# CederGroupHub/chgnet

Measured on AMD Instinct MI355X. Metric: structures/s (energy+force+stress) on batched ~50-atom crystals, higher is better.
Workload: dtype f32; 1 GPU; 1024 x LiMnO2 5x1x1 (40 atoms, sigma=0.01 frac perturbation) per GPU, task efs; structures_per_gpu=1024, atoms=40960, directed_bonds=3535504, angles=4125764, bond_graph_nodes=213755, weights=random-init 0.3.0 architecture (tests/golden/weights_seed0.npz), parallelism=structures sharded over 1 GPU(s), RCCL all-gather of energies only, process_group_ranks=1, energies_in_all_gather=1024, comm=none (single rank)

## Files before the change

### chgnet_amd/_lib.py

```python

from __future__ import annotations

import ctypes
import os

c_int_p = ctypes.POINTER(ctypes.c_int32)
c_float_p = ctypes.POINTER(ctypes.c_float)

TASK_BITS = {"e": 1, "f": 2, "s": 4, "m": 8}

EXPORTED_SYMBOLS = (
    "chg_abi_version", "chg_device_count", "chg_weights_required", "chg_engine_create", "chg_engine_destroy", "chg_last_error",
    "chg_batch_upload", "chg_batch_build", "chg_batch_build_predict", "chg_debug_fetch_i32", "chg_batch_update_geometry", "chg_batch_free", "chg_batch_device_bytes",
    "chg_predict", "chg_synchronize", "chg_batch_download", "chg_timer_start", "chg_timer_stop_ms",
    "chg_profile_enable", "chg_profile_reset", "chg_profile_count", "chg_profile_read",
    "chg_debug_fetch", "chg_test_rows_gemm", "chg_test_split_gemm",
    "chg_engine_set_memory_limit", "chg_engine_memory_info", "chg_batch_bytes_required",
    "chg_stream_copy", "chg_backward", "chg_engine_build_stats", "chg_engine_update_weights",
    "chg_engine_set_graph_search", "chg_engine_cell_stats",
    "chg_comm_unique_id", "chg_comm_create", "chg_comm_all_gather_f32", "chg_comm_all_reduce_sum_f32", "chg_comm_barrier",
    "chg_comm_destroy", "chg_comm_last_error",
    "chg_comm_all_gather_f32_device", "chg_comm_all_reduce_sum_f32_device", "chg_comm_reserve", "chg_comm_info",
    "chg_backward_allreduce", "chg_batch_all_gather_energy", "chg_engine_stream", "chg_engine_device",
    "chg_host_alloc", "chg_host_free",
    "chg_relax_create", "chg_relax_run", "chg_relax_download", "chg_relax_free", "chg_test_relax_step",
    "chg_relax_create_lbfgs", "chg_test_lbfgs_step",
    "chg_md_create", "chg_md_run", "chg_md_download", "chg_md_free", "chg_test_md_step",
    "chg_md_create_langevin", "chg_test_md_step_langevin",
    "chg_md_create_nhc", "chg_md_download_nhc", "chg_test_md_step_nhc",
    "chg_md_create_nhc_flex", "chg_md_download_vg", "chg_test_md_step_nhc_flex",
    "chg_hessian_vector", "chg_hessian_vector_strain",
# ... 173 lines not shown
    lib.chg_batch_all_gather_energy.argtypes = [vp, vp, vp, ctypes.c_int64, c_float_p]
    lib.chg_engine_stream.argtypes = [vp]
    lib.chg_engine_stream.restype = ctypes.c_void_p
    lib.chg_engine_device.argtypes = [vp]
    lib.chg_engine_update_weights.argtypes = [vp, c_float_p]
    lib.chg_batch_download.argtypes = [vp, vp, ctypes.POINTER(OutHost)]
    lib.chg_timer_start.argtypes = [vp]
    lib.chg_timer_stop_ms.argtypes = [vp, c_float_p]
    lib.chg_stream_copy.argtypes = [vp, ctypes.c_int64, ctypes.c_int, c_float_p]
    lib.chg_profile_enable.argtypes = [vp, ctypes.c_int]
    lib.chg_profile_reset.argtypes = [vp]
    lib.chg_profile_count.argtypes = [vp]
    lib.chg_profile_read.argtypes = [vp, ctypes.c_int, ctypes.c_char_p, ctypes.c_int, ctypes.POINTER(ctypes.c_int64), ctypes.POINTER(ctypes.c_double)]
    lib.chg_debug_fetch.argtypes = [vp, vp, ctypes.c_char_p, c_float_p, ctypes.c_int64, ctypes.POINTER(ctypes.c_int64)]
    lib.chg_test_rows_gemm.argtypes = [vp, c_float_p, c_float_p, c_float_p, c_float_p, ctypes.c_int, ctypes.c_int, ctypes.c_int]
    lib.chg_test_split_gemm.argtypes = [vp, c_float_p, c_float_p, c_float_p, ctypes.c_int, ctypes.c_int, ctypes.c_int]
    dp = ctypes.POINTER(ctypes.c_double)
    lib.chg_relax_create.argtypes = [vp, ctypes.POINTER(StructsHost), ctypes.POINTER(RelaxParams), ctypes.POINTER(vp)]
    lib.chg_relax_run.argtypes = [vp, vp, ctypes.c_int32, c_int_p]
    lib.chg_relax_download.argtypes = [vp, vp, ctypes.POINTER(RelaxOutHost)]
    lib.chg_relax_free.argtypes = [vp, vp]
    lib.chg_test_relax_step.argtypes = [vp, ctypes.POINTER(RelaxParams), ctypes.c_int32, c_int_p, dp, dp, dp, c_int_p, c_float_p, c_float_p,
                                        c_float_p, c_float_p, dp, dp]
    lib.chg_relax_create_lbfgs.argtypes = [vp, ctypes.POINTER(StructsHost), ctypes.POINTER(RelaxParams), ctypes.POINTER(LbfgsParams),
                                           ctypes.POINTER(vp)]
    lib.chg_test_lbfgs_step.argtypes = [vp, ctypes.POINTER(RelaxParams), ctypes.POINTER(LbfgsParams), ctypes.c_int32, c_int_p, dp, dp, dp, dp, dp,
                                        dp, dp, c_int_p, c_float_p, c_float_p, c_float_p, c_float_p, ctypes.c_int32, dp, dp, c_int_p]
    lib.chg_md_create.argtypes = [vp, ctypes.POINTER(StructsHost), dp, dp, ctypes.POINTER(MdParams), ctypes.POINTER(vp)]
    lib.chg_md_run.argtypes = [vp, vp, ctypes.c_int32]
    lib.chg_md_download.argtypes = [vp, vp, ctypes.POINTER(MdOutHost)]
    lib.chg_md_free.argtypes = [vp, vp]
# ... 34 lines not shown
```

### chgnet_amd/csrc/engine.hip

```cpp

#include "engine_internal.h"
#include <cstring>

namespace chgh {

template <int UNROLL>
__global__ __launch_bounds__(256) void k_stream_copy(const f32x4* __restrict__ src, f32x4* __restrict__ dst, size_t n) {
  const size_t stride = (size_t)gridDim.x * blockDim.x;
  size_t i = (size_t)blockIdx.x * blockDim.x + threadIdx.x;
  for (; i + (UNROLL - 1) * stride < n; i += UNROLL * stride) {
    f32x4 v[UNROLL];
#pragma unroll
    for (int u = 0; u < UNROLL; ++u) v[u] = __builtin_nontemporal_load(src + i + u * stride);
#pragma unroll
    for (int u = 0; u < UNROLL; ++u) __builtin_nontemporal_store(v[u], dst + i + u * stride);
  }
  for (; i < n; i += stride) dst[i] = src[i];
}

template <bool NT>
__global__ __launch_bounds__(256) void k_stream_copy_seg(const f32x4* __restrict__ src, f32x4* __restrict__ dst, size_t n) {
  constexpr size_t SEG = 1024;
  const size_t nseg = n / SEG;
  for (size_t sgm = blockIdx.x; sgm < nseg; sgm += gridDim.x) {
// ... 542 lines not shown
  float *dx = nullptr, *dw = nullptr, *db = nullptr, *dy = nullptr;
  HIP_TRY(eng, hipMalloc(&dx, sizeof(float) * (size_t)rows * k));
  HIP_TRY(eng, hipMalloc(&dw, sizeof(float) * (size_t)nout * k));
  HIP_TRY(eng, hipMalloc(&db, sizeof(float) * (size_t)nout));
  HIP_TRY(eng, hipMalloc(&dy, sizeof(float) * (size_t)rows * nout));
  HIP_TRY(eng, hipMemcpy(dx, x, sizeof(float) * (size_t)rows * k, hipMemcpyHostToDevice));
  HIP_TRY(eng, hipMemcpy(dw, wt, sizeof(float) * (size_t)nout * k, hipMemcpyHostToDevice));
  if (bias) HIP_TRY(eng, hipMemcpy(db, bias, sizeof(float) * (size_t)nout, hipMemcpyHostToDevice));
  int s = rows_gemm(eng, "test_gemm", k, nout, dx, k, nullptr, dw, bias ? db : nullptr, nullptr, 0, dy, nout, nullptr, rows, 0);
  if (s == CHG_OK && hipStreamSynchronize(eng->stream) != hipSuccess) { eng->err = "test gemm failed"; s = CHG_EHIP; }
  if (s == CHG_OK) hipMemcpy(y, dy, sizeof(float) * (size_t)rows * nout, hipMemcpyDeviceToHost);
  hipFree(dx); hipFree(dw); hipFree(db); hipFree(dy);
  return s;
}

int chg_test_split_gemm(chg_engine* eng, const float* x, const float* w, float* y, int rows, int f, int mode) {
  if (!eng || !x || !w || !y || rows <= 0 || (f != D && f != 2 * D) || mode < 0 || mode > 3) return CHG_EINVAL;
  HIP_TRY(eng, hipSetDevice(eng->device));
  const int kin = (mode & 1) ? f : D, nout = (mode & 1) ? D : f;
  float *dx = nullptr, *dw = nullptr, *dy = nullptr;
  HIP_TRY(eng, hipMalloc(&dx, sizeof(float) * (size_t)rows * kin));
  HIP_TRY(eng, hipMalloc(&dw, sizeof(float) * (size_t)f * D));
  HIP_TRY(eng, hipMalloc(&dy, sizeof(float) * (size_t)rows * nout));
  HIP_TRY(eng, hipMemcpy(dx, x, sizeof(float) * (size_t)rows * kin, hipMemcpyHostToDevice));
  HIP_TRY(eng, hipMemcpy(dw, w, sizeof(float) * (size_t)f * D, hipMemcpyHostToDevice));
  hipStream_t st = eng->stream;
  switch (mode * 2 + (f == D ? 0 : 1)) {
    case 0: launch_test_split<0, D>(st, dx, dw, dy, rows); break;
    case 1: launch_test_split<0, 2 * D>(st, dx, dw, dy, rows); break;
    case 2: launch_test_split<1, D>(st, dx, dw, dy, rows); break;
// ... 15 lines not shown
```

### chgnet_amd/csrc/engine_internal.h

```cpp
#pragma once

#include "chgnet_hip.h"

#include <hip/hip_runtime.h>

#include <algorithm>
#include <cmath>
#include <cstdint>
#include <cstdio>
#include <cstdlib>
#include <cstring>
#include <functional>
#include <map>
#include <mutex>
#include <string>
#include <unordered_map>
#include <vector>

#include "mfma_tile.h"
#include "mfma_split.h"
#include "kernels_conv.h"
#include "kernels_angle_w.h"
#include "kernels_angle_blk.h"
#include "kernels_embed.h"
// ... 24 lines not shown
  }
  std::string& slot() const { return texts()[this]; }
  ErrText& operator=(const std::string& v) { slot() = v; return *this; }
  ErrText& operator=(const char* v) { slot() = v; return *this; }
  operator std::string() const { return slot(); }
  const char* c_str() const { return slot().c_str(); }
  ~ErrText() { texts().erase(this); }
};
inline std::string operator+(const char* a, const ErrText& b) { return std::string(a) + std::string(b); }
inline std::string operator+(const std::string& a, const ErrText& b) { return a + std::string(b); }
inline std::string operator+(const ErrText& a, const char* b) { return std::string(a) + b; }
inline std::string operator+(const ErrText& a, const std::string& b) { return std::string(a) + b; }

struct ProfEntry { std::string label; int64_t launches = 0; double ms = 0.0; };
struct PendingEvent { int entry; hipEvent_t start, stop; };

struct chg_engine {
  int device = 0;
  hipStream_t stream = nullptr;
  chg_model_desc desc{};
  float* d_weights = nullptr;
  Weights w{};
  float* d_images = nullptr;
  const float* p_elem = nullptr;
  const float* img_ac_fwd[2][MAX_CONV] = {};
  const float* img_ac_bwd_rm[MAX_CONV] = {};
  const float* img_angle[2][2 * MAX_CONV] = {};
  ErrText err;
  hipEvent_t t0 = nullptr, t1 = nullptr;
  bool profiling = false;
// ... 10 lines not shown
  bool force_wide = false;
  char* scratch = nullptr;
  size_t scratch_bytes = 0, scratch_wanted = 0;
  char* h_stage = nullptr;
  size_t h_stage_bytes = 0;
  char* h_out = nullptr;
  size_t h_out_bytes = 0;
  int num_cus = 256;
  bool spec_builds = true;
  int last_N = 0, last_Ed = 0, last_A = 0, last_Eb = 0;
  double last_r_atom = 0.0, last_r_bond = 0.0;
  long n_spec_builds = 0, n_spec_overflows = 0, n_cell_builds = 0, n_cell_fallbacks = 0;
  int graph_search = 0;
  int cell_min_atoms = 2048;
  size_t memory_limit = 0;
};

struct Train2;

struct chg_batch {
  int B = 0, N = 0, Ed = 0, Eu = 0, A = 0, Eb = 0, L = 0;
  char* arena = nullptr;
  size_t arena_bytes = 0;
  int *z, *atom_owner, *atom_off, *e_center, *e_nbr, *e_d2u, *e_owner, *e_rev, *p_center, *p_nbr, *u_u2d, *u_bnode, *bn_und, *a_ctr, *a_b1c, *a_b2c, *a_d1, *a_d2;
  float *frac, *lattice, *e_image;
  float* cart;
  f32x4 *ev, *eu;
  float *hb0, *wag, *wbgc;
  float* atom[MAX_CONV + 1];
  float* hbc[MAX_CONV + 1];
// ... 194 lines not shown
```

### chgnet_amd/csrc/engine_predict.hip

```cpp
#include "engine_internal.h"

#include "kernels_geom.h"
#include "kernels_angle_fa.h"
#include "kernels_chain.h"

namespace chgh {


struct Cursor {
  const float* base;
  size_t pos = 0;
  const float* take(size_t n) {
    pos += (4 - pos % 4) % 4;
    const float* p = base + pos;
    pos += n;
    return p;
  }
};

void take_gated_tail(Cursor& c, GatedW& g, const float*& w2c_t, const float*& w2g_t) {
  g.w2c = c.take(D * D); g.b2c = c.take(D); g.w2g = c.take(D * D); g.b2g = c.take(D);
  w2c_t = c.take(D * D); w2g_t = c.take(D * D);
}
void take_ln(Cursor& c, GatedW& g) {
// ... 73 lines not shown
constexpr int EMBED_GRID_MULT = 2;

int grid_for(int rows, int max_blocks, int block_rows) {
  int ntiles = (rows + block_rows - 1) / block_rows;
  int g = std::min(ntiles, max_blocks);
  if (g >= 8) g &= ~7;
  return std::max(g, 1);
}

int tile_grid(chg_engine* eng, int rows, int block_rows) {
  const int ntiles = (rows + block_rows - 1) / block_rows;
  const int mult = ntiles <= 4 * eng->num_cus ? 1 : TILE_GRID_MULT;
  return std::max(1, std::min((ntiles + 7) & ~7, mult * eng->num_cus));
}

template <int K, int NOUT, int PARTS = 1>
int launch_rows_gemm(chg_engine* eng, const char* label, const RowsGemm& p) {
  if (p.rows <= 0) return CHG_OK;
  LaunchScope ls(eng, label);
  const size_t lds = rows_gemm_lds<K, NOUT, PARTS>();
  hipLaunchKernelGGL((k_rows_gemm<K, NOUT, PARTS>), dim3(grid_for(p.rows, 4 * eng->num_cus)), dim3(BLOCK), lds, eng->stream, p);
  HIP_TRY(eng, hipGetLastError());
  return CHG_OK;
}

constexpr int SMALL_GEMM_ROWS = 32768;
constexpr int SMALL_GEMM_COLS = 16;
template <int K, int PARTS>
int launch_rows_gemm_cols(chg_engine* eng, const char* label, RowsGemm p, int n_out, int n_out_first) {
  if (p.rows <= 0) return CHG_OK;
  p.col_blocks = n_out / SMALL_GEMM_COLS; p.blocks1 = n_out_first / SMALL_GEMM_COLS;
  LaunchScope ls(eng, label);
  hipLaunchKernelGGL((k_rows_gemm<K, SMALL_GEMM_COLS, PARTS>), dim3(grid_for(p.rows, 4 * eng->num_cus), p.col_blocks), dim3(BLOCK),
                     (rows_gemm_lds<K, SMALL_GEMM_COLS, PARTS>()), eng->stream, p);
  HIP_TRY(eng, hipGetLastError());
  return CHG_OK;
}

int rows_gemm(chg_engine* eng, const char* label, int K, int NOUT, const float* X, int ldx, const int* in_idx, const float* Wt,
              const float* bias, const float* resid, int ldr, float* Y, int ldy, const int* out_idx, int rows, int accumulate) {
  RowsGemm p{X, ldx, in_idx, Wt, bias, resid, ldr, Y, ldy, out_idx, rows, accumulate, nullptr, 0, 0, 0, 0};
  if (rows <= SMALL_GEMM_ROWS && K == 64 && (NOUT == 64 || NOUT == 128)) return launch_rows_gemm_cols<64, 1>(eng, label, p, NOUT, NOUT);
  if (rows <= SMALL_GEMM_ROWS && K == 128 && NOUT == 64) return launch_rows_gemm_cols<128, 1>(eng, label, p, NOUT, NOUT);
  if (K == 64 && NOUT == 64) return launch_rows_gemm<64, 64>(eng, label, p);
  if (K == 64 && NOUT == 128) return launch_rows_gemm<64, 128>(eng, label, p);
  if (K == 128 && NOUT == 64) return launch_rows_gemm<128, 64>(eng, label, p);
  eng->err = "rows_gemm: unsupported shape";
  return CHG_EINVAL;
}

int rows_gemm_out2(chg_engine* eng, const char* label, const float* X, const int* in_idx, const float* Wt, const float* Wt2,
                   const float* bias, float* Y, int ldy, int rows) {
  RowsGemm p{X, D, in_idx, Wt, bias, nullptr, 0, Y, ldy, nullptr, rows, 0, Wt2, 0, 2 * D, 0, 0};
  if (rows <= SMALL_GEMM_ROWS) return launch_rows_gemm_cols<64, 1>(eng, label, p, 4 * D, 2 * D);
  return launch_rows_gemm<64, 128, 2>(eng, label, p);
}
int rows_gemm_in2(chg_engine* eng, const char* label, const float* X, int ldx, const float* Wt, const float* Wt2, float* Y,
                  const int* out_idx, int rows, int accumulate) {
  RowsGemm p{X, ldx, nullptr, Wt, nullptr, nullptr, 0, Y, D, out_idx, rows, accumulate, Wt2, 2 * D, 0, 0, 0};
  if (rows <= SMALL_GEMM_ROWS) return launch_rows_gemm_cols<128, 2>(eng, label, p, D, D);
  return launch_rows_gemm<128, 64, 2>(eng, label, p);
}

struct MultiGemm {
  RowsGemmN g{};
  int max_rows = 0;
  void add(RowsGemm p, int n_out, int n_out_first) {
    p.col_blocks = n_out / SMALL_GEMM_COLS; p.blocks1 = n_out_first / SMALL_GEMM_COLS;
    g.p[g.n++] = p;
    max_rows = std::max(max_rows, p.rows);
  }
};
template <int K>
int launch_rows_gemm_multi(chg_engine* eng, const char* label, const MultiGemm& m) {
  int blocks = 0;
  for (int i = 0; i < m.g.n; ++i) blocks += m.g.p[i].col_blocks;
  LaunchScope ls(eng, label);
  hipLaunchKernelGGL((k_rows_gemm_multi<K, SMALL_GEMM_COLS>), dim3(grid_for(m.max_rows, 4 * eng->num_cus), blocks), dim3(BLOCK),
                     (rows_gemm_lds<K, SMALL_GEMM_COLS, (K == 128 ? 2 : 1)>()), eng->stream, m.g);
  HIP_TRY(eng, hipGetLastError());
  return CHG_OK;
}
static bool small_rows(int rows) { return rows > 0 && rows <= SMALL_GEMM_ROWS; }

int zero(chg_engine* eng, void* p, size_t bytes) {
  if (bytes == 0) return CHG_OK;
  LaunchScope ls(eng, "memset");
  HIP_TRY(eng, hipMemsetAsync(p, 0, bytes, eng->stream));
  return CHG_OK;
}





static bool addr32_mode(const chg_batch* b) {
  constexpr size_t HARD = (size_t)1 << 32;
  static const int forced = [] { const char* e = std::getenv("CHGNET_ADDR_MODE"); return e ? std::atoi(e) : 0; }();
// ... 136 lines not shown
  return CHG_OK;
}

int atomconv_bwd(chg_engine* eng, chg_batch* b, int l) {
  const ACW& w = eng->w.ac[l];
  if (b->Ed == 0) return CHG_OK;
  TRY(rows_gemm(eng, "gemm_Gagg", 64, 64, b->Ga, D, nullptr, w.w_out_t, nullptr, nullptr, 0, b->GA, D, nullptr, b->N, 0));
  TRY(atomconv_bwd_kernel(eng, b, l));
  if (l > 0) TRY(rows_gemm_in2(eng, "gemm_GP", b->GP_l[l], 4 * D, w.w_cn_t, w.w_cn_t + 2 * D * D, b->Ga, nullptr, b->N, 1));
  return CHG_OK;
}

int angle_tables(chg_engine* eng, chg_batch* b, int slot, const float* atom, const float* hbc, const float* w_bij, const float* w_ctr, const float* b1,
                 int p_layer = -1) {
  float *S = b->Sl[slot], *R = b->Rl[slot];
  if (small_rows(b->N) && small_rows(b->Eb)) {
    MultiGemm m;
    m.add(RowsGemm{atom, D, nullptr, w_ctr, b1, nullptr, 0, S, 2 * D, nullptr, b->N, 0, nullptr, 0, 0, 0, 0}, 2 * D, 2 * D);
    m.add(RowsGemm{hbc, D, nullptr, w_bij, nullptr, nullptr, 0, R, 4 * D, nullptr, b->Eb, 0, w_bij + 2 * D * D, 0, 2 * D, 0, 0}, 4 * D, 2 * D);
    if (p_layer >= 0 && b->Ed > 0) {
      m.add(atomconv_p_problem(eng, b, p_layer), 4 * D, 2 * D);
      b->p_table_done = p_layer;
    }
    return launch_rows_gemm_multi<64>(eng, m.g.n == 3 ? "gemm_SRP" : "gemm_SR", m);
  }
  TRY(rows_gemm(eng, "gemm_S", 64, 128, atom, D, nullptr, w_ctr, b1, nullptr, 0, S, 2 * D, nullptr, b->N, 0));
  return rows_gemm_out2(eng, "gemm_R", hbc, nullptr, w_bij, w_bij + 2 * D * D, nullptr, R, 4 * D, b->Eb);
}

AngleArgs angle_args(chg_batch* b, int slot, const float* ang, const float* w_ang, const GatedW& g, float* out) {
  AngleArgs a{};
// ... 68 lines not shown

int bondconv_fwd(chg_engine* eng, chg_batch* b, int l) {
  const BCW& w = eng->w.bc[l];
  TRY(angle_tables(eng, b, l, b->atom[l + 1], b->hbc[l], w.w_bij, w.w_ctr, w.b1, l + 1));
  TRY((launch_angle<true, false>(eng, "bondconv_fwd", b, angle_args(b, l, b->ang[l], w.w_ang, w.g, b->aggB_l[l]))));
  return rows_gemm(eng, "gemm_out", 64, 64, b->aggB_l[l], D, nullptr, w.w_out, w.b_out, b->hbc[l], D, b->hbc[l + 1], D, nullptr, b->Eb, 0);
}

int angleupd_fwd(chg_engine* eng, chg_batch* b, int l) {
  const AUW& w = eng->w.au[l];
  TRY(angle_tables(eng, b, b->L + l, b->atom[l + 1], b->hbc[l + 1], w.w_bij, w.w_ctr, w.b1));
  return launch_angle<false, false, FWD_WAVES>(eng, "angleupd_fwd", b, angle_args(b, b->L + l, b->ang[l], w.w_ang, w.g, b->ang[l + 1]));
}

int angle_table_grads(chg_engine* eng, chg_batch* b, int slot, const float* w_bij_t, const float* w_ctr_t) {
  if (small_rows(b->N) && small_rows(b->Eb)) {
    MultiGemm m;
    m.add(RowsGemm{b->GR_l[slot], 4 * D, nullptr, w_bij_t, nullptr, nullptr, 0, b->Gb, D, b->bn_und, b->Eb, 1, w_bij_t + 2 * D * D, 2 * D, 0, 0, 0}, D, D);
    m.add(RowsGemm{b->GS_l[slot], 2 * D, nullptr, w_ctr_t, nullptr, nullptr, 0, b->Ga, D, nullptr, b->N, 1, nullptr, 0, 0, 0, 0}, D, D);
    return launch_rows_gemm_multi<128>(eng, "gemm_GRS", m);
  }
  TRY(rows_gemm_in2(eng, "gemm_GR", b->GR_l[slot], 4 * D, w_bij_t, w_bij_t + 2 * D * D, b->Gb, b->bn_und, b->Eb, 1));
  return rows_gemm(eng, "gemm_GS", 128, 64, b->GS_l[slot], 2 * D, nullptr, w_ctr_t, nullptr, nullptr, 0, b->Ga, D, nullptr, b->N, 1);
}

int bondconv_bwd(chg_engine* eng, chg_batch* b, int l) {
  const BCW& w = eng->w.bc[l];
  TRY(rows_gemm(eng, "gemm_Gagg", 64, 64, b->Gb, D, b->bn_und, w.w_out_t, nullptr, nullptr, 0, b->Gagg, D, nullptr, b->Eb, 0));
  TRY((launch_angle<true, true>(eng, "bondconv_bwd", b, angle_args(b, l, b->ang[l], w.w_ang, w.g, nullptr))));
  return angle_table_grads(eng, b, l, w.w_bij_t, w.w_ctr_t);
}
// ... 451 lines not shown
  return CHG_OK;
}

void register_names(chg_batch* b) {
  auto& m = b->named;
  m.clear();
  const size_t N = b->N, Ed = b->Ed, Eu = b->Eu, A = b->A, Eb = b->Eb, B = b->B;
  m["cart"] = {b->cart, 3 * N};
  m["ev"] = {reinterpret_cast<const float*>(b->ev), 4 * Ed};
  m["eu"] = {reinterpret_cast<const float*>(b->eu), 4 * Ed};
  m["hb0"] = {b->hb0, Eu * D}; m["wag"] = {b->wag, Eu * D}; m["wbgc"] = {b->wbgc, Eb * D};
  for (int l = 0; l <= b->L; ++l) m["atom" + std::to_string(l)] = {b->atom[l], N * D};
  for (int l = 0; l < b->L; ++l) m["hbc" + std::to_string(l)] = {b->hbc[l], Eb * D};
  for (int l = 0; l < b->L - 1; ++l) m["ang" + std::to_string(l)] = {b->ang[l], A * D};
  for (int l = 0; l < b->L; ++l) { m["P" + std::to_string(l)] = {b->Pl[l], N * 4 * D}; m["Q" + std::to_string(l)] = {b->Ql[l], Eu * 2 * D}; }
  m["agg"] = {b->agg_l[b->L - 1], N * D}; m["aggB"] = {b->aggB_l[0], Eb * D};
  m["Ga"] = {b->Ga, N * D}; m["GA"] = {b->GA, N * D}; m["Gb"] = {b->Gb, Eu * D}; m["Gwag"] = {b->Gwag, Eu * D};
  m["Gwbgc"] = {b->Gwbgc, Eb * D}; m["Gang"] = {b->Gang, A * D}; m["GP"] = {b->GP_l[0], N * 4 * D}; m["GQ"] = {b->GQ, Eu * 2 * D};
  m["GR"] = {b->GR_l[0], Eb * 4 * D}; m["GS"] = {b->GS_l[0], N * 2 * D}; m["Grk"] = {b->Grk, Eu}; m["Gu"] = {b->Gu, 4 * Ed};
  m["virial"] = {b->virial, 9 * B}; m["volume"] = {b->volume, B};
  m["frac"] = {b->frac, 3 * N}; m["lattice"] = {b->lattice, 9 * B}; m["e_image"] = {b->e_image, 3 * Ed};
  auto& mi = b->named_i32;
  mi.clear();
  mi["z"] = {b->z, N}; mi["atom_owner"] = {b->atom_owner, N}; mi["atom_off"] = {b->atom_off, B + 1};
  mi["e_center"] = {b->e_center, Ed}; mi["e_nbr"] = {b->e_nbr, Ed}; mi["e_d2u"] = {b->e_d2u, Ed}; mi["e_owner"] = {b->e_owner, Ed};
  mi["e_rev"] = {b->e_rev, Ed}; mi["p_center"] = {b->p_center, Ed}; mi["p_nbr"] = {b->p_nbr, Ed};
  mi["u_u2d"] = {b->u_u2d, Eu}; mi["u_bnode"] = {b->u_bnode, Eu}; mi["bn_und"] = {b->bn_und, Eb};
  mi["a_ctr"] = {b->a_ctr, A}; mi["a_b1c"] = {b->a_b1c, A}; mi["a_b2c"] = {b->a_b2c, A}; mi["a_d1"] = {b->a_d1, A}; mi["a_d2"] = {b->a_d2, A};
  mi["win_flag"] = {b->win.flag, 4}; mi["win_q_a"] = {b->win.q_a, A}; mi["win_q_ctr"] = {b->win.q_ctr, A}; mi["win_na"] = {b->win.na, N + 1};
  mi["win_aoff"] = {b->win.aoff, N + 1}; mi["win_q_ab1"] = {b->win.q_ab1, A}; mi["win_q_ab2"] = {b->win.q_ab2, A};
  mi["win_next_atom"] = {b->win.next_atom, A ? N : 0};
  mi["blk_tiles"] = {b->blk_tiles, b->blk_cap ? (size_t)1 : 0}; mi["blk_a"] = {b->blk_a, (size_t)b->blk_cap * TILE_ROWS};
  mi["blk_b1c"] = {b->blk_b1c, (size_t)b->blk_cap * TILE_ROWS}; mi["blk_b2c"] = {b->blk_b2c, (size_t)b->blk_cap * TILE_ROWS};
  mi["blk_ctr"] = {b->blk_ctr, (size_t)b->blk_cap * TILE_ROWS}; mi["blk_desc"] = {b->blk_desc, (size_t)b->blk_cap};
  mi["win_wave_head"] = {b->win.wave_head, A ? (size_t)WIN_MAX_GRID * WAVES : 0}; mi["win_xatom"] = {b->win.xatom, (size_t)WIN_MAX_GRID / 8 + 1};
}


int predict_set_lds(chg_engine* eng) {
  int s;
  if ((s = set_lds(eng, k_rows_gemm<64, 64>, rows_gemm_lds<64, 64>()))) return s;
  if ((s = set_lds(eng, k_rows_gemm<64, 128>, rows_gemm_lds<64, 128>()))) return s;
  if ((s = set_lds(eng, k_rows_gemm<128, 64>, rows_gemm_lds<128, 64>()))) return s;
  if ((s = set_lds(eng, k_rows_gemm<64, SMALL_GEMM_COLS, 1>, (rows_gemm_lds<64, SMALL_GEMM_COLS, 1>())))) return s;
  if ((s = set_lds(eng, k_rows_gemm_multi<64, SMALL_GEMM_COLS>, (rows_gemm_lds<64, SMALL_GEMM_COLS, 1>())))) return s;
  if ((s = set_lds(eng, k_rows_gemm_multi<128, SMALL_GEMM_COLS>, (rows_gemm_lds<128, SMALL_GEMM_COLS, 2>())))) return s;
  if ((s = set_lds(eng, k_rows_gemm<128, SMALL_GEMM_COLS, 1>, (rows_gemm_lds<128, SMALL_GEMM_COLS, 1>())))) return s;
  if ((s = set_lds(eng, k_rows_gemm<128, SMALL_GEMM_COLS, 2>, (rows_gemm_lds<128, SMALL_GEMM_COLS, 2>())))) return s;
  if ((s = set_lds(eng, (k_rows_gemm<64, 128, 2>), (rows_gemm_lds<64, 128, 2>())))) return s;
  if ((s = set_lds(eng, (k_rows_gemm<128, 64, 2>), (rows_gemm_lds<128, 64, 2>())))) return s;
  if ((s = set_lds(eng, k_atomconv_fwd<FWD_WAVES>, (atomconv_lds<FWD_WAVES, false, true>())))) return s;
  if ((s = set_lds(eng, k_atomconv_bwd<false>, acb_fused_lds()))) return s;
  if ((s = set_lds(eng, k_angleupd_fwd_a<>, angle_fa_lds()))) return s;
  if ((s = set_lds(eng, (k_atomconv_fwd<FWD_WAVES, true>), (atomconv_lds<FWD_WAVES, false, true>())))) return s;
  if ((s = set_lds(eng, (k_atomconv_bwd<false, true>), acb_fused_lds()))) return s;
  if ((s = set_lds(eng, k_angleupd_fwd_a<true>, angle_fa_lds()))) return s;
  if ((s = set_lds(eng, (k_angle_bwd_w<true, false, false, true>), angle_w_lds<true>()))) return s;
  if ((s = set_lds(eng, (k_angle_bwd_w<true, false, true, true>), angle_w_lds<true>()))) return s;
  if ((s = set_lds(eng, (k_angle_bwd_w<false, false, false, true>), angle_w_lds<false>()))) return s;
  if ((s = set_lds(eng, (k_angle<true, false, WAVES, false, true>), angle_lds<true>()))) return s;
  if ((s = set_lds(eng, k_angle_bwd_blk<true>, angle_blk_lds<true>()))) return s;
  if ((s = set_lds(eng, k_angle_bwd_blk<false>, angle_blk_lds<false>()))) return s;
  if ((s = set_lds(eng, k_angle_bwd_w<true>, angle_w_lds<true>()))) return s;
  if ((s = set_lds(eng, k_angle_bwd_w<false>, angle_w_lds<false>()))) return s;
  if ((s = set_lds(eng, (k_angle_bwd_w<true, true>), angle_w_lds<true>()))) return s;
// ... 23 lines not shown
```

### chgnet_amd/csrc/kernels_conv.h

```cpp
#pragma once

#include "mfma_tile.h"
#include "mfma_split.h"

namespace chg {

constexpr int TS = 2 * D + PAD;
constexpr int WS = D + PAD;
constexpr int TILE_FLOATS = TILE_ROWS * TS;
constexpr int VEC_SLOTS = 6;
constexpr int IMG64 = 1024, IMG128 = 2048;
constexpr int angle_split(bool hidden, bool bwd) { return (hidden && bwd) ? 2 : 1; }

struct GatedW {
  const float *w2c, *b2c, *w2g, *b2g, *ln1_g, *ln1_b, *ln2_g, *ln2_b;
};

__device__ __forceinline__ void stage_gated_vecs(float* vecs, const GatedW& gw, bool hidden, int tid) {
  if (hidden) {
    stage_vector(vecs + 0 * D, gw.b2c, D, tid);
    stage_vector(vecs + 1 * D, gw.b2g, D, tid);
  }
  stage_vector(vecs + 2 * D, gw.ln1_g, D, tid);
  stage_vector(vecs + 3 * D, gw.ln1_b, D, tid);
// ... 352 lines not shown
#pragma unroll
  for (int i = 0; i < 3; ++i) {
    if (i >= g.n) return;
    if (y < g.p[i].col_blocks) {
      if (K == 128 && g.p[i].x2_off > 0) rows_gemm_body<K, NOUT, (K == 128 ? 2 : 1)>(g.p[i], y);
      else rows_gemm_body<K, NOUT, 1>(g.p[i], y);
      return;
    }
    y -= g.p[i].col_blocks;
  }
}

template <int K, int NOUT, int PARTS = 1>
constexpr size_t rows_gemm_lds() {
  return sizeof(float) * (PARTS * NOUT * (K + PAD) + NOUT + WAVES * TILE_ROWS * ((K > NOUT ? K : NOUT) + PAD));
}

struct AtomConvArgs {
  const float* P;
  const float* Q;
  const float* wag;
  const int *e_center, *e_nbr, *e_d2u;
  int n_edges;
  GatedW gw;
  const float *hb0, *hbc;
  const int* u_bnode;
  const float *w_bond, *q_bias;
  float* Qout;
  const float* image;
  float* agg;
// ... 707 lines not shown
```

### chgnet_amd/engine.py

```python

from __future__ import annotations

import ctypes
import weakref

import numpy as np

from chgnet_amd import _lib
from chgnet_amd.graph.structure import atomic_numbers_of
from chgnet_amd.pack import D, PackedBatch, PackedWeights, _check_z, pack_batch


def _fp(a: np.ndarray):
    return a.ctypes.data_as(_lib.c_float_p)


def _ip(a: np.ndarray):
    return a.ctypes.data_as(_lib.c_int_p)


class PreparedStructures:

    __slots__ = ("n_struct", "z", "atom_off", "frac", "lattice")

# ... 325 lines not shown
        got = ctypes.c_int64()
        self._check(self.lib.chg_debug_fetch(self.handle, batch.handle, name.encode(), _fp(dst), n, ctypes.byref(got)))
        if got.value != n:
            raise RuntimeError(f"debug_fetch({name}): expected {n} floats, device buffer has {got.value}")
        return dst[:n].reshape(shape)

    def test_split_gemm(self, x: np.ndarray, w: np.ndarray, mode: int) -> np.ndarray:
        x = np.ascontiguousarray(x, np.float32)
        w = np.ascontiguousarray(w, np.float32)
        f = w.shape[0]
        assert w.shape[1] == 64 and x.shape[1] == (f if mode & 1 else 64)
        y = np.empty((x.shape[0], 64 if mode & 1 else f), np.float32)
        self._check(self.lib.chg_test_split_gemm(self.handle, _fp(x), _fp(w), _fp(y), x.shape[0], f, int(mode)))
        return y

    def test_rows_gemm(self, x: np.ndarray, wt: np.ndarray, bias: np.ndarray | None) -> np.ndarray:
        x = np.ascontiguousarray(x, np.float32)
        wt = np.ascontiguousarray(wt, np.float32)
        rows, k = x.shape
        nout = wt.shape[0]
        y = np.empty((rows, nout), np.float32)
        b = np.ascontiguousarray(bias, np.float32) if bias is not None else None
        self._check(self.lib.chg_test_rows_gemm(self.handle, _fp(x), _fp(wt), _fp(b) if b is not None else None, _fp(y), rows, k, nout))
        return y
```

### include/chgnet_hip.h

```cpp
#ifndef CHGNET_HIP_H
#define CHGNET_HIP_H

#include <stdint.h>

#ifdef __cplusplus
extern "C" {
#endif

typedef enum {
  CHG_OK = 0,
  CHG_EINVAL = -1,
  CHG_EHIP = -2,
  CHG_ENOMEM = -3,
  CHG_ENODEV = -4,
  CHG_EUNSUPPORTED = -5,
  CHG_ERANGE = -6
} chg_status;

enum {
  CHG_TASK_E = 1u,
  CHG_TASK_F = 2u,
  CHG_TASK_S = 4u,
  CHG_TASK_M = 8u
};
// ... 101 lines not shown
int chg_batch_download(chg_engine* eng, chg_batch* batch, const chg_out_host* out);

int chg_timer_start(chg_engine* eng);
int chg_timer_stop_ms(chg_engine* eng, float* elapsed_ms);

int chg_stream_copy(chg_engine* eng, int64_t bytes, int iters, float* ms_per_iter);

int chg_profile_enable(chg_engine* eng, int on);
int chg_profile_reset(chg_engine* eng);
int chg_profile_count(chg_engine* eng);
int chg_profile_read(chg_engine* eng, int i, char* label, int label_cap, int64_t* launches, double* total_ms);

int chg_debug_fetch(chg_engine* eng, chg_batch* batch, const char* name, float* dst, int64_t capacity, int64_t* n_written);

int chg_test_rows_gemm(chg_engine* eng, const float* x, const float* wt, const float* bias, float* y, int rows, int k, int nout);
int chg_test_split_gemm(chg_engine* eng, const float* x, const float* w, float* y, int rows, int f, int mode);

enum { CHG_RELAX_RUNNING = 0, CHG_RELAX_CONVERGED = 1, CHG_RELAX_MAX_STEPS = 2, CHG_RELAX_NONFINITE = 3 };
typedef struct chg_relax_params {
  double fmax;
  int32_t max_steps, relax_cell;
  double dt, maxstep, dtmax, finc, fdec, astart, fa;
  int32_t nmin;
  double exp_cell_factor;
  double r_atom, r_bond, numerical_tol;
  double stress_weight;
} chg_relax_params;
typedef struct chg_relax chg_relax;
typedef struct chg_relax_out_host {
  double* frac;
// ... 153 lines not shown
```

Before: 41040 structures/s.

## Add software-pipelined persistent rows GEMM kernel for large row counts

```diff
diff --git a/chgnet_amd/_lib.py b/chgnet_amd/_lib.py
--- a/chgnet_amd/_lib.py
+++ b/chgnet_amd/_lib.py
@@ -14,7 +14,7 @@
     "chg_batch_upload", "chg_batch_build", "chg_batch_build_predict", "chg_debug_fetch_i32", "chg_batch_update_geometry", "chg_batch_free", "chg_batch_device_bytes",
     "chg_predict", "chg_synchronize", "chg_batch_download", "chg_timer_start", "chg_timer_stop_ms",
     "chg_profile_enable", "chg_profile_reset", "chg_profile_count", "chg_profile_read",
-    "chg_debug_fetch", "chg_test_rows_gemm", "chg_test_split_gemm",
+    "chg_debug_fetch", "chg_test_rows_gemm", "chg_test_split_gemm", "chg_test_set_gemm_stream_rows",
     "chg_engine_set_memory_limit", "chg_engine_memory_info", "chg_batch_bytes_required",
     "chg_stream_copy", "chg_backward", "chg_engine_build_stats", "chg_engine_update_weights",
     "chg_engine_set_graph_search", "chg_engine_cell_stats",
@@ -218,7 +218,8 @@
     lib.chg_profile_read.argtypes = [vp, ctypes.c_int, ctypes.c_char_p, ctypes.c_int, ctypes.POINTER(ctypes.c_int64), ctypes.POINTER(ctypes.c_double)]
     lib.chg_debug_fetch.argtypes = [vp, vp, ctypes.c_char_p, c_float_p, ctypes.c_int64, ctypes.POINTER(ctypes.c_int64)]
     lib.chg_test_rows_gemm.argtypes = [vp, c_float_p, c_float_p, c_float_p, c_float_p, ctypes.c_int, ctypes.c_int, ctypes.c_int]
-    lib.chg_test_split_gemm.argtypes = [vp, c_float_p, c_float_p, c_float_p, ctypes.c_int, ctypes.c_int, ctypes.c_int]
+    lib.chg_test_set_gemm_stream_rows.argtypes = [vp, ctypes.c_int]
+    lib.chg_test_split_gemm.argtypes =[vp, c_float_p, c_float_p, c_float_p, ctypes.c_int, ctypes.c_int, ctypes.c_int]
     dp = ctypes.POINTER(ctypes.c_double)
     lib.chg_relax_create.argtypes = [vp, ctypes.POINTER(StructsHost), ctypes.POINTER(RelaxParams), ctypes.POINTER(vp)]
     lib.chg_relax_run.argtypes = [vp, vp, ctypes.c_int32, c_int_p]
diff --git a/chgnet_amd/csrc/engine.hip b/chgnet_amd/csrc/engine.hip
--- a/chgnet_amd/csrc/engine.hip
+++ b/chgnet_amd/csrc/engine.hip
@@ -580,6 +580,12 @@
   return s;
 }
 
+int chg_test_set_gemm_stream_rows(chg_engine* eng, int rows) {
+  if (!eng) return CHG_EINVAL;
+  eng->gemm_stream_rows = rows < 0 ? SMALL_GEMM_ROWS : rows;
+  return CHG_OK;
+}
+
 int chg_test_split_gemm(chg_engine* eng, const float* x, const float* w, float* y, int rows, int f, int mode) {
   if (!eng || !x || !w || !y || rows <= 0 || (f != D && f != 2 * D) || mode < 0 || mode > 3) return CHG_EINVAL;
   HIP_TRY(eng, hipSetDevice(eng->device));
diff --git a/chgnet_amd/csrc/engine_internal.h b/chgnet_amd/csrc/engine_internal.h
--- a/chgnet_amd/csrc/engine_internal.h
+++ b/chgnet_amd/csrc/engine_internal.h
@@ -62,6 +62,8 @@
 
 struct ProfEntry { std::string label; int64_t launches = 0; double ms = 0.0; };
 struct PendingEvent { int entry; hipEvent_t start, stop; };
+
+constexpr int SMALL_GEMM_ROWS = 32768;
 
 struct chg_engine {
   int device = 0;
@@ -102,6 +104,7 @@
   int graph_search = 0;
   int cell_min_atoms = 2048;
   size_t memory_limit = 0;
+  int gemm_stream_rows = SMALL_GEMM_ROWS;
 };
 
 struct Train2;
diff --git a/chgnet_amd/csrc/engine_predict.hip b/chgnet_amd/csrc/engine_predict.hip
--- a/chgnet_amd/csrc/engine_predict.hip
+++ b/chgnet_amd/csrc/engine_predict.hip
@@ -111,17 +111,33 @@
   return std::max(1, std::min((ntiles + 7) & ~7, mult * eng->num_cus));
 }
 
+constexpr int STREAM_GRID_MULT = 1;
 template <int K, int NOUT, int PARTS = 1>
-int launch_rows_gemm(chg_engine* eng, const char* label, const RowsGemm& p) {
+int launch_rows_gemm_stream(chg_engine* eng, const char* label, const RowsGemm& p) {
   if (p.rows <= 0) return CHG_OK;
   LaunchScope ls(eng, label);
   const size_t lds = rows_gemm_lds<K, NOUT, PARTS>();
-  hipLaunchKernelGGL((k_rows_gemm<K, NOUT, PARTS>), dim3(grid_for(p.rows, 4 * eng->num_cus)), dim3(BLOCK), lds, eng->stream, p);
+  const dim3 grid(grid_for(p.rows, STREAM_GRID_MULT * eng->num_cus));
+  const int rmw = (p.accumulate ? 1 : 0) | (p.resid ? 2 : 0);
+  if (PARTS == 2 && (rmw > 1 || (K == 64 && rmw))) { eng->err = "rows_gemm: unsupported two-part form"; return CHG_EINVAL; }
+  if (rmw == 0) hipLaunchKernelGGL((k_rows_gemm_stream<K, NOUT, PARTS, 0>), grid, dim3(BLOCK), lds, eng->stream, p);
+  else if (rmw == 1) hipLaunchKernelGGL((k_rows_gemm_stream<K, NOUT, (K == 64 ? 1 : PARTS), 1>), grid, dim3(BLOCK), lds, eng->stream, p);
+  else if (rmw == 2) hipLaunchKernelGGL((k_rows_gemm_stream<K, NOUT, 1, 2>), grid, dim3(BLOCK), lds, eng->stream, p);
+  else hipLaunchKernelGGL((k_rows_gemm_stream<K, NOUT, 1, 3>), grid, dim3(BLOCK), lds, eng->stream, p);
   HIP_TRY(eng, hipGetLastError());
   return CHG_OK;
 }
 
-constexpr int SMALL_GEMM_ROWS = 32768;
+template <int K, int NOUT>
+int set_lds_stream(chg_engine* eng) {
+  int s;
+  if ((s = set_lds(eng, (k_rows_gemm_stream<K, NOUT, 1, 0>), (rows_gemm_lds<K, NOUT, 1>())))) return s;
+  if ((s = set_lds(eng, (k_rows_gemm_stream<K, NOUT, 1, 1>), (rows_gemm_lds<K, NOUT, 1>())))) return s;
+  if ((s = set_lds(eng, (k_rows_gemm_stream<K, NOUT, 1, 2>), (rows_gemm_lds<K, NOUT, 1>())))) return s;
+  if ((s = set_lds(eng, (k_rows_gemm_stream<K, NOUT, 1, 3>), (rows_gemm_lds<K, NOUT, 1>())))) return s;
+  return CHG_OK;
+}
+
 constexpr int SMALL_GEMM_COLS = 16;
 template <int K, int PARTS>
 int launch_rows_gemm_cols(chg_engine* eng, const char* label, RowsGemm p, int n_out, int n_out_first) {
@@ -137,11 +153,11 @@
 int rows_gemm(chg_engine* eng, const char* label, int K, int NOUT, const float* X, int ldx, const int* in_idx, const float* Wt,
               const float* bias, const float* resid, int ldr, float* Y, int ldy, const int* out_idx, int rows, int accumulate) {
   RowsGemm p{X, ldx, in_idx, Wt, bias, resid, ldr, Y, ldy, out_idx, rows, accumulate, nullptr, 0, 0, 0, 0};
-  if (rows <= SMALL_GEMM_ROWS && K == 64 && (NOUT == 64 || NOUT == 128)) return launch_rows_gemm_cols<64, 1>(eng, label, p, NOUT, NOUT);
-  if (rows <= SMALL_GEMM_ROWS && K == 128 && NOUT == 64) return launch_rows_gemm_cols<128, 1>(eng, label, p, NOUT, NOUT);
-  if (K == 64 && NOUT == 64) return launch_rows_gemm<64, 64>(eng, label, p);
-  if (K == 64 && NOUT == 128) return launch_rows_gemm<64, 128>(eng, label, p);
-  if (K == 128 && NOUT == 64) return launch_rows_gemm<128, 64>(eng, label, p);
+  if (rows <= eng->gemm_stream_rows && K == 64 && (NOUT == 64 || NOUT == 128)) return launch_rows_gemm_cols<64, 1>(eng, label, p, NOUT, NOUT);
+  if (rows <= eng->gemm_stream_rows && K == 128 && NOUT == 64) return launch_rows_gemm_cols<128, 1>(eng, label, p, NOUT, NOUT);
+  if (K == 64 && NOUT == 64) return launch_rows_gemm_stream<64, 64>(eng, label, p);
+  if (K == 64 && NOUT == 128) return launch_rows_gemm_stream<64, 128>(eng, label, p);
+  if (K == 128 && NOUT == 64) return launch_rows_gemm_stream<128, 64>(eng, label, p);
   eng->err = "rows_gemm: unsupported shape";
   return CHG_EINVAL;
 }
@@ -149,14 +165,14 @@
 int rows_gemm_out2(chg_engine* eng, const char* label, const float* X, const int* in_idx, const float* Wt, const float* Wt2,
                    const float* bias, float* Y, int ldy, int rows) {
   RowsGemm p{X, D, in_idx, Wt, bias, nullptr, 0, Y, ldy, nullptr, rows, 0, Wt2, 0, 2 * D, 0, 0};
-  if (rows <= SMALL_GEMM_ROWS) return launch_rows_gemm_cols<64, 1>(eng, label, p, 4 * D, 2 * D);
-  return launch_rows_gemm<64, 128, 2>(eng, label, p);
+  if (rows <= eng->gemm_stream_rows) return launch_rows_gemm_cols<64, 1>(eng, label, p, 4 * D, 2 * D);
+  return launch_rows_gemm_stream<64, 128, 2>(eng, label, p);
 }
 int rows_gemm_in2(chg_engine* eng, const char* label, const float* X, int ldx, const float* Wt, const float* Wt2, float* Y,
                   const int* out_idx, int rows, int accumulate) {
   RowsGemm p{X, ldx, nullptr, Wt, nullptr, nullptr, 0, Y, D, out_idx, rows, accumulate, Wt2, 2 * D, 0, 0, 0};
-  if (rows <= SMALL_GEMM_ROWS) return launch_rows_gemm_cols<128, 2>(eng, label, p, D, D);
-  return launch_rows_gemm<128, 64, 2>(eng, label, p);
+  if (rows <= eng->gemm_stream_rows) return launch_rows_gemm_cols<128, 2>(eng, label, p, D, D);
+  return launch_rows_gemm_stream<128, 64, 2>(eng, label, p);
 }
 
 struct MultiGemm {
@@ -178,7 +194,7 @@
   HIP_TRY(eng, hipGetLastError());
   return CHG_OK;
 }
-static bool small_rows(int rows) { return rows > 0 && rows <= SMALL_GEMM_ROWS; }
+static bool small_rows(chg_engine* eng, int rows) { return rows > 0 && rows <= eng->gemm_stream_rows; }
 
 int zero(chg_engine* eng, void* p, size_t bytes) {
   if (bytes == 0) return CHG_OK;
@@ -345,7 +361,7 @@
 int angle_tables(chg_engine* eng, chg_batch* b, int slot, const float* atom, const float* hbc, const float* w_bij, const float* w_ctr, const float* b1,
                  int p_layer = -1) {
   float *S = b->Sl[slot], *R = b->Rl[slot];
-  if (small_rows(b->N) && small_rows(b->Eb)) {
+  if (small_rows(eng, b->N) && small_rows(eng, b->Eb)) {
     MultiGemm m;
     m.add(RowsGemm{atom, D, nullptr, w_ctr, b1, nullptr, 0, S, 2 * D, nullptr, b->N, 0, nullptr, 0, 0, 0, 0}, 2 * D, 2 * D);
     m.add(RowsGemm{hbc, D, nullptr, w_bij, nullptr, nullptr, 0, R, 4 * D, nullptr, b->Eb, 0, w_bij + 2 * D * D, 0, 2 * D, 0, 0}, 4 * D, 2 * D);
@@ -444,7 +460,7 @@
 }
 
 int angle_table_grads(chg_engine* eng, chg_batch* b, int slot, const float* w_bij_t, const float* w_ctr_t) {
-  if (small_rows(b->N) && small_rows(b->Eb)) {
+  if (small_rows(eng, b->N) && small_rows(eng, b->Eb)) {
     MultiGemm m;
     m.add(RowsGemm{b->GR_l[slot], 4 * D, nullptr, w_bij_t, nullptr, nullptr, 0, b->Gb, D, b->bn_und, b->Eb, 1, w_bij_t + 2 * D * D, 2 * D, 0, 0, 0}, D, D);
     m.add(RowsGemm{b->GS_l[slot], 2 * D, nullptr, w_ctr_t, nullptr, nullptr, 0, b->Ga, D, nullptr, b->N, 1, nullptr, 0, 0, 0, 0}, D, D);
@@ -926,6 +942,7 @@
   for (int l = 0; l < b->L; ++l) m["hbc" + std::to_string(l)] = {b->hbc[l], Eb * D};
   for (int l = 0; l < b->L - 1; ++l) m["ang" + std::to_string(l)] = {b->ang[l], A * D};
   for (int l = 0; l < b->L; ++l) { m["P" + std::to_string(l)] = {b->Pl[l], N * 4 * D}; m["Q" + std::to_string(l)] = {b->Ql[l], Eu * 2 * D}; }
+  m["R"] = {b->Rl[0], Eb * 4 * D}; m["S"] = {b->Sl[0], N * 2 * D};
   m["agg"] = {b->agg_l[b->L - 1], N * D}; m["aggB"] = {b->aggB_l[0], Eb * D};
   m["Ga"] = {b->Ga, N * D}; m["GA"] = {b->GA, N * D}; m["Gb"] = {b->Gb, Eu * D}; m["Gwag"] = {b->Gwag, Eu * D};
   m["Gwbgc"] = {b->Gwbgc, Eb * D}; m["Gang"] = {b->Gang, A * D}; m["GP"] = {b->GP_l[0], N * 4 * D}; m["GQ"] = {b->GQ, Eu * 2 * D};
@@ -951,16 +968,15 @@
 
 int predict_set_lds(chg_engine* eng) {
   int s;
-  if ((s = set_lds(eng, k_rows_gemm<64, 64>, rows_gemm_lds<64, 64>()))) return s;
-  if ((s = set_lds(eng, k_rows_gemm<64, 128>, rows_gemm_lds<64, 128>()))) return s;
-  if ((s = set_lds(eng, k_rows_gemm<128, 64>, rows_gemm_lds<128, 64>()))) return s;
+  if ((s = set_lds_stream<64, 64>(eng)) || (s = set_lds_stream<64, 128>(eng)) || (s = set_lds_stream<128, 64>(eng))) return s;
   if ((s = set_lds(eng, k_rows_gemm<64, SMALL_GEMM_COLS, 1>, (rows_gemm_lds<64, SMALL_GEMM_COLS, 1>())))) return s;
   if ((s = set_lds(eng, k_rows_gemm_multi<64, SMALL_GEMM_COLS>, (rows_gemm_lds<64, SMALL_GEMM_COLS, 1>())))) return s;
   if ((s = set_lds(eng, k_rows_gemm_multi<128, SMALL_GEMM_COLS>, (rows_gemm_lds<128, SMALL_GEMM_COLS, 2>())))) return s;
   if ((s = set_lds(eng, k_rows_gemm<128, SMALL_GEMM_COLS, 1>, (rows_gemm_lds<128, SMALL_GEMM_COLS, 1>())))) return s;
   if ((s = set_lds(eng, k_rows_gemm<128, SMALL_GEMM_COLS, 2>, (rows_gemm_lds<128, SMALL_GEMM_COLS, 2>())))) return s;
-  if ((s = set_lds(eng, (k_rows_gemm<64, 128, 2>), (rows_gemm_lds<64, 128, 2>())))) return s;
-  if ((s = set_lds(eng, (k_rows_gemm<128, 64, 2>), (rows_gemm_lds<128, 64, 2>())))) return s;
+  if ((s = set_lds(eng, (k_rows_gemm_stream<64, 128, 2, 0>), (rows_gemm_lds<64, 128, 2>())))) return s;
+  if ((s = set_lds(eng, (k_rows_gemm_stream<128, 64, 2, 0>), (rows_gemm_lds<128, 64, 2>())))) return s;
+  if ((s = set_lds(eng, (k_rows_gemm_stream<128, 64, 2, 1>), (rows_gemm_lds<128, 64, 2>())))) return s;
   if ((s = set_lds(eng, k_atomconv_fwd<FWD_WAVES>, (atomconv_lds<FWD_WAVES, false, true>())))) return s;
   if ((s = set_lds(eng, k_atomconv_bwd<false>, acb_fused_lds()))) return s;
   if ((s = set_lds(eng, k_angleupd_fwd_a<>, angle_fa_lds()))) return s;
diff --git a/chgnet_amd/csrc/kernels_conv.h b/chgnet_amd/csrc/kernels_conv.h
--- a/chgnet_amd/csrc/kernels_conv.h
+++ b/chgnet_amd/csrc/kernels_conv.h
@@ -390,6 +390,128 @@
 template <int K, int NOUT, int PARTS = 1>
 constexpr size_t rows_gemm_lds() {
   return sizeof(float) * (PARTS * NOUT * (K + PAD) + NOUT + WAVES * TILE_ROWS * ((K > NOUT ? K : NOUT) + PAD));
+}
+
+template <int K, int NOUT, int PARTS, int RMW>
+__device__ __forceinline__ void rows_gemm_stream_body(const RowsGemm& p) {
+  extern __shared__ __attribute__((aligned(16))) float smem[];
+  constexpr bool IN2 = PARTS == 2 && K > NOUT, OUT2 = PARTS == 2 && !IN2;
+  static_assert(NOUT % 64 == 0 && (PARTS == 1 || PARTS == 2), "full-width instances only");
+  constexpr int KS = K + PAD, KT = K / 16, NFT = NOUT / 16;
+  constexpr int XS = (K > NOUT ? K : NOUT) + PAD;
+  constexpr int XP = IN2 ? 2 : 1, YP = OUT2 ? 2 : 1;
+  float* W = smem;
+  float* bias = W + PARTS * NOUT * KS;
+  float* tiles = bias + NOUT;
+  const int tid = threadIdx.x, wave = tid >> 6, lane = tid & 63, j = lane & 15, g = lane >> 4;
+  stage_split<false>(reinterpret_cast<h16x8*>(W), p.Wt, NOUT, K, tid, BLOCK);
+  if (PARTS == 2) stage_split<false>(reinterpret_cast<h16x8*>(W + NOUT * KS), p.Wt2, NOUT, K, tid, BLOCK);
+  for (int idx = tid; idx < NOUT; idx += BLOCK) bias[idx] = p.bias ? p.bias[idx] : 0.f;
+  __syncthreads();
+  float* T = tiles + wave * TILE_ROWS * XS;
+  const int ntiles = (p.rows + BLOCK_ROWS - 1) / BLOCK_ROWS;
+  int tb, te;
+  tile_range(ntiles, tb, te);
+  constexpr int LPR = K / 4, RPS = 64 / LPR, NV = TILE_ROWS / RPS;
+  constexpr int LPO = NOUT / 4, RPO = 64 / LPO, NO = TILE_ROWS / RPO;
+  const int subx = lane / LPR, tx = lane % LPR, suby = lane / LPO, ty = lane % LPO;
+  auto rows_of = [&](int tile, int& nvalid, int& in_row, int& out_row) {
+    const int row0 = tile * BLOCK_ROWS + wave * TILE_ROWS;
+    nvalid = tile < te ? min(TILE_ROWS, p.rows - row0) : 0;
+    const int rr_ = nvalid > 0 ? row0 + (j < nvalid ? j : 0) : 0;
+    in_row = p.in_idx ? p.in_idx[rr_] : rr_;
+    out_row = p.out_idx ? p.out_idx[rr_] : rr_;
+  };
+  auto issue_x = [&](int in_row, f32x4 (&v)[XP][NV]) {
+#pragma unroll
+    for (int xp = 0; xp < XP; ++xp) {
+      const float* X = p.X + (xp ? p.x2_off : 0);
+#pragma unroll
+      for (int it = 0; it < NV; ++it) {
+        const int r = __shfl(in_row, RPS * it + subx);
+        v[xp][it] = *reinterpret_cast<const f32x4*>(X + (size_t)r * p.ldx + 4 * tx);
+      }
+    }
+  };
+  auto to_lds = [&](const f32x4 (&v)[NV]) {
+#pragma unroll
+    for (int it = 0; it < NV; ++it) *reinterpret_cast<f32x4*>(T + (RPS * it + subx) * XS + 4 * tx) = v[it];
+    __builtin_amdgcn_wave_barrier();
+  };
+  f32x4 vn[XP][NV], x[KT];
+  auto take_x = [&]() {
+    to_lds(vn[0]);
+    read_dl<KT>(T + j * XS, g, x);
+    __builtin_amdgcn_wave_barrier();
+    if constexpr (IN2) to_lds(vn[1]);
+  };
+  int nvalid_c, in_c, out_c, nvalid_n, in_n, out_n;
+  rows_of(tb, nvalid_c, in_c, out_c);
+  rows_of(tb + 1, nvalid_n, in_n, out_n);
+  issue_x(in_c, vn);
+  take_x();
+  for (int tile = tb; tile < te && nvalid_c > 0; ++tile) {
+    const int out_row = out_c, in_next = in_n;
+    nvalid_c = nvalid_n; out_c = out_n;
+    rows_of(tile + 2, nvalid_n, in_n, out_n);
+    int orow[NO];
+#pragma unroll
+    for (int it = 0; it < NO; ++it) orow[it] = __shfl(out_row, RPO * it + suby);
+    f32x4 old[YP][NO];
+    if constexpr (RMW != 0) {
+#pragma unroll
+      for (int yp = 0; yp < YP; ++yp)
+#pragma unroll
+        for (int it = 0; it < NO; ++it) {
+          if (RMW & 1) old[yp][it] = *reinterpret_cast<const f32x4*>(p.Y + (yp ? p.y2_off : 0) + (size_t)orow[it] * p.ldy + 4 * ty);
+          if (RMW == 2) old[yp][it] = *reinterpret_cast<const f32x4*>(p.resid + (yp ? p.y2_off : 0) + (size_t)orow[it] * p.ldr + 4 * ty);
+          if (RMW == 3) old[yp][it] += *reinterpret_cast<const f32x4*>(p.resid + (yp ? p.y2_off : 0) + (size_t)orow[it] * p.ldr + 4 * ty);
+        }
+    }
+    issue_x(in_next, vn);
+    __builtin_amdgcn_sched_barrier(0);
+    f32x4 ov[YP][NO];
+#pragma unroll
+    for (int yp = 0; yp < YP; ++yp) {
+      f32x4 acc[NFT];
+      if (yp == 0) {
+        read_dl<NFT>(bias, g, acc);
+      } else {
+#pragma unroll
+        for (int ft = 0; ft < NFT; ++ft) acc[ft] = zero4();
+      }
+      gemm_split<KT, NFT, true>(acc, reinterpret_cast<const h16x8*>(W + yp * NOUT * KS), NOUT, x, j, g);
+      if constexpr (IN2) {
+        read_dl<KT>(T + j * XS, g, x);
+        __builtin_amdgcn_wave_barrier();
+        gemm_split<KT, NFT, true>(acc, reinterpret_cast<const h16x8*>(W + NOUT * KS), NOUT, x, j, g);
+      }
+      write_dl<NFT>(T + j * XS, g, acc);
+      __builtin_amdgcn_wave_barrier();
+#pragma unroll
+      for (int it = 0; it < NO; ++it) {
+        ov[yp][it] = *reinterpret_cast<const f32x4*>(T + (RPO * it + suby) * XS + 4 * ty);
+        if constexpr (RMW != 0) ov[yp][it] += old[yp][it];
+      }
+      __builtin_amdgcn_wave_barrier();
+    }
+#pragma unroll
+    for (int yp = 0; yp < YP; ++yp)
+#pragma unroll
+      for (int it = 0; it < NO; ++it) asm volatile("" : "+v"(ov[yp][it]));
+#pragma unroll
+    for (int yp = 0; yp < YP; ++yp)
+#pragma unroll
+      for (int it = 0; it < NO; ++it)
+        *reinterpret_cast<f32x4*>(p.Y + (yp ? p.y2_off : 0) + (size_t)orow[it] * p.ldy + 4 * ty) = ov[yp][it];
+    take_x();
+    asm volatile("" : "+v"(in_n), "+v"(out_n));
+  }
+}
+
+template <int K, int NOUT, int PARTS, int RMW>
+__global__ __launch_bounds__(BLOCK) CHG_TWO_WAVES void k_rows_gemm_stream(RowsGemm p) {
+  rows_gemm_stream_body<K, NOUT, PARTS, RMW>(p);
 }
 
 struct AtomConvArgs {
diff --git a/chgnet_amd/engine.py b/chgnet_amd/engine.py
--- a/chgnet_amd/engine.py
+++ b/chgnet_amd/engine.py
@@ -363,6 +363,9 @@
         self._check(self.lib.chg_test_split_gemm(self.handle, _fp(x), _fp(w), _fp(y), x.shape[0], f, int(mode)))
         return y
 
+    def test_set_gemm_stream_rows(self, rows: int) -> None:
+        self._check(self.lib.chg_test_set_gemm_stream_rows(self.handle, int(rows)))
+
     def test_rows_gemm(self, x: np.ndarray, wt: np.ndarray, bias: np.ndarray | None) -> np.ndarray:
         x = np.ascontiguousarray(x, np.float32)
         wt = np.ascontiguousarray(wt, np.float32)
diff --git a/include/chgnet_hip.h b/include/chgnet_hip.h
--- a/include/chgnet_hip.h
+++ b/include/chgnet_hip.h
@@ -139,6 +139,7 @@
 int chg_debug_fetch(chg_engine* eng, chg_batch* batch, const char* name, float* dst, int64_t capacity, int64_t* n_written);
 
 int chg_test_rows_gemm(chg_engine* eng, const float* x, const float* wt, const float* bias, float* y, int rows, int k, int nout);
+int chg_test_set_gemm_stream_rows(chg_engine* eng, int rows);
 int chg_test_split_gemm(chg_engine* eng, const float* x, const float* w, float* y, int rows, int f, int mode);
 
 enum { CHG_RELAX_RUNNING = 0, CHG_RELAX_CONVERGED = 1, CHG_RELAX_MAX_STEPS = 2, CHG_RELAX_NONFINITE = 3 };
```

Result: no change. 41420 structures/s, median of 6 (+0.9%).
